# sun-huangqingbo/multiplexed-image-annotator

Measured on AMD Instinct MI355X. Metric: cells/sec annotated (whole node), higher is better.
Workload: dtype f16

## Files before the change

multiplexed-image-annotator_amd/csrc/cell_attention.hip:

```cpp

#include "gemm_epi.h"
#include "ribca_common.h"
#include "ribca_kernels.h"

namespace ribca {

namespace {

typedef __attribute__((__vector_size__(4 * sizeof(_Float16)))) _Float16 f16x4c;
typedef __attribute__((__vector_size__(4 * sizeof(short)))) short s16x4c;
__device__ __forceinline__ f16x4c lds_read_tr16c(const char* p) {
  return __builtin_bit_cast(f16x4c, __builtin_amdgcn_ds_read_tr16_b64_v4i16((s16x4c __attribute__((address_space(3)))*)(p)));
}

constexpr int kTP = 112, kVRows = 128;

template <int D, int HD> struct CellGeom {
  static constexpr int Dp = (D + 31) / 32 * 32;
  static constexpr int NK = Dp / 32;
  static constexpr int GD = HD == 32 ? 64 : 48;
  static constexpr int NTP = GD / 16;
  static constexpr int WROWS = 3 * GD;
  static constexpr int WSTAGE = WROWS * ROWB;
  static constexpr int GROUPS = D / GD;
  static constexpr int HPG = GD / HD;
  static constexpr int KIMG = kTP * ROWB;
  static constexpr int VROWB = 4 * GD;
  static constexpr int VIMG = kVRows * VROWB + 64;
  static constexpr int CB = 2 * 3 * D * 4;
  static constexpr int RING = 3;
  static constexpr int OFF_K = RING * WSTAGE;
  static constexpr int OFF_V = OFF_K + HPG * KIMG;
  static constexpr int OFF_CB = OFF_V + (VIMG + 15) / 16 * 16;
  static constexpr int LDS = OFF_CB + CB;
  static_assert(D % GD == 0 && GD % HD == 0 && HD % 4 == 0 && HD <= 32 && HPG % 2 == 0 && WROWS % 8 == 0, "head geometry");
};

}

template <int D, int HD>
__global__ __launch_bounds__(512) void cell_qkv_attention_kernel(const uint16_t* __restrict__ z, int ldz, const uint16_t* __restrict__ W, int ldw,
                                                                 const float* __restrict__ bias2, const float* __restrict__ csum,
                                                                 const float2* __restrict__ rowstat, uint16_t* __restrict__ out, int ldo, int T,
                                                                 float scale) {
  using G = CellGeom<D, HD>;
  constexpr int NK = G::NK, GROUPS = G::GROUPS, HPG = G::HPG, kRing = G::RING, kGroupDims = G::GD, NTP = G::NTP, kWStage = G::WSTAGE;
  constexpr int NTILES = 3 * NTP;
  constexpr int TOTAL = GROUPS * NK;
  constexpr int GPL = G::WROWS / 8;
  extern __shared__ __attribute__((aligned(16))) char smem[];
  const int tid = threadIdx.x, lane = tid & 63;
  const int wave = __builtin_amdgcn_readfirstlane(tid >> 6);
  const int cell = blockIdx.x;
  const int r16 = lane & 15, g = lane >> 4;

  for (int i = tid; i < 3 * D / 4; i += 512) {
    reinterpret_cast<float4*>(smem + G::OFF_CB)[i] = reinterpret_cast<const float4*>(csum)[i];
    reinterpret_cast<float4*>(smem + G::OFF_CB + 3 * D * 4)[i] = reinterpret_cast<const float4*>(bias2)[i];
  }
  for (int o = kTP * G::VROWB + tid * 16; o < G::VIMG; o += 512 * 16) *reinterpret_cast<uint4*>(smem + G::OFF_V + o) = uint4{0u, 0u, 0u, 0u};
  __syncthreads();

  if (wave == 7) {
    auto issue = [&](int step) {
      const int hg = step / NK, s = step - hg * NK;
      char* st = smem + (step % kRing) * kWStage;
#pragma unroll
      for (int i = 0; i < GPL; ++i) {
        const int row = i * 8 + (lane >> 3);
        const int which = row / kGroupDims, c = row - which * kGroupDims;
        const int n = which * D + hg * kGroupDims + c;
        const int ch = (lane & 7) ^ swz_f(row);
        const uint16_t* src = W + (size_t)n * ldw + s * (2 * BK) + ch * 8;
        __builtin_amdgcn_global_load_lds((const __attribute__((address_space(1))) void*)src, (__attribute__((address_space(3))) void*)(st + i * 1024), 16,
                                         0, 0);
      }
    };
    issue(0);
    issue(1);
    for (int step = 0; step < TOTAL; ++step) {
      if (step + 1 < TOTAL) wait_vmcnt<GPL>();
      else wait_vmcnt<0>();
      __builtin_amdgcn_s_barrier();
      asm volatile("" ::: "memory");
      if (step + 2 < TOTAL) issue(step + 2);
      if ((step + 1) % NK == 0) __builtin_amdgcn_s_barrier();
    }
    return;
  }

  const int tok = wave * 16 + r16;
  const int trow = tok < T ? tok : T - 1;
  const uint16_t* zr = z + ((size_t)cell * T + trow) * ldz;
  f16x8 ahi[NK], alo[NK];
#pragma unroll
  for (int s = 0; s < NK; ++s) {
    const uint4* p = reinterpret_cast<const uint4*>(zr + (4 * s + g) * 16);
    ahi[s] = __builtin_bit_cast(f16x8, p[0]);
    alo[s] = __builtin_bit_cast(f16x8, p[1]);
  }
  const float2 rs = rowstat[(size_t)cell * T + trow];
  const float rstd = rs.x, nm = -rs.y * rs.x;
  const char* cb = smem + G::OFF_CB;
  uint16_t* orow = out + ((size_t)cell * T + tok) * ldo;
  int w_rd[NTILES];
#pragma unroll
  for (int j = 0; j < NTILES; ++j) w_rd[j] = lds_off(16 * j + r16, 2 * g);
  const int k_wr = lds_off(tok, 2 * g);
  constexpr int KST = 4, NT = 7;

  int step = 0;
  for (int hg = 0; hg < GROUPS; ++hg) {
    f32x4 acc[NTILES];
#pragma unroll
    for (int j = 0; j < NTILES; ++j) acc[j] = f32x4{0.f, 0.f, 0.f, 0.f};
#pragma unroll
    for (int s = 0; s < NK; ++s, ++step) {
      asm volatile("s_waitcnt lgkmcnt(0)" ::: "memory");
      __builtin_amdgcn_s_barrier();
      asm volatile("" ::: "memory");
      const char* st = smem + (step % kRing) * kWStage;
#pragma unroll
      for (int jb = 0; jb < NTILES / 3; ++jb) {
        f16x8 whi[3], wlo[3];
#pragma unroll
        for (int j = 0; j < 3; ++j) {
          whi[j] = __builtin_bit_cast(f16x8, *reinterpret_cast<const uint4*>(st + w_rd[3 * jb + j]));
          wlo[j] = __builtin_bit_cast(f16x8, *reinterpret_cast<const uint4*>(st + (w_rd[3 * jb + j] ^ 16)));
        }
#pragma unroll
        for (int j = 0; j < 3; ++j) acc[3 * jb + j] = mfma_f16(wlo[j], ahi[s], acc[3 * jb + j]);
#pragma unroll
        for (int j = 0; j < 3; ++j) acc[3 * jb + j] = mfma_f16(whi[j], alo[s], acc[3 * jb + j]);
#pragma unroll
        for (int j = 0; j < 3; ++j) acc[3 * jb + j] = mfma_f16(whi[j], ahi[s], acc[3 * jb + j]);
      }
    }
#pragma unroll
    for (int j = 0; j < NTILES; ++j) {
      const int n = (j / NTP) * D + hg * kGroupDims + 16 * (j % NTP) + 4 * g;
      const float4 c4 = *reinterpret_cast<const float4*>(cb + n * 4), b4 = *reinterpret_cast<const float4*>(cb + 3 * D * 4 + n * 4);
      const f32x2v r2 = {rstd, rstd}, n2 = {nm, nm};
      const f32x2v lo2 = fma2(r2, f32x2v{acc[j][0], acc[j][1]}, fma2(n2, f32x2v{c4.x, c4.y}, f32x2v{b4.x, b4.y}));
      const f32x2v hi2 = fma2(r2, f32x2v{acc[j][2], acc[j][3]}, fma2(n2, f32x2v{c4.z, c4.w}, f32x2v{b4.z, b4.w}));
      acc[j] = f32x4{lo2.x, lo2.y, hi2.x, hi2.y};
    }
    f16x8 qhi[HPG], qlo[HPG];
#pragma unroll
    for (int h = 0; h < HPG; ++h) {
      constexpr int dummy = 0; (void)dummy;
      const int d_lo = h * HD, d_hi = d_lo + HD;
      const int tA = d_lo / 16, tB = (d_hi - 1) / 16;
      const bool inA = 16 * tA + 4 * g >= d_lo && 16 * tA + 4 * g < d_hi;
      const bool inB = tB != tA && 16 * tB + 4 * g >= d_lo && 16 * tB + 4 * g < d_hi;
      float qa[4], qb[4], ka[4], kb[4];
#pragma unroll
      for (int r = 0; r < 4; ++r) {
        qa[r] = inA ? acc[tA][r] * scale : 0.f;
        qb[r] = inB ? acc[tB][r] * scale : 0.f;
        ka[r] = inA ? acc[NTP + tA][r] : 0.f;
        kb[r] = inB ? acc[NTP + tB][r] : 0.f;
      }
      uint2 h0, l0, h1, l1;
      split4(qa, h0, l0);
      split4(qb, h1, l1);
      qhi[h] = __builtin_bit_cast(f16x8, uint4{h0.x, h0.y, h1.x, h1.y});
      qlo[h] = __builtin_bit_cast(f16x8, uint4{l0.x, l0.y, l1.x, l1.y});
      split4(ka, h0, l0);
      split4(kb, h1, l1);
      char* kimg = smem + G::OFF_K + h * G::KIMG;
      *reinterpret_cast<uint4*>(kimg + k_wr) = uint4{h0.x, h0.y, h1.x, h1.y};
      *reinterpret_cast<uint4*>(kimg + (k_wr ^ 16)) = uint4{l0.x, l0.y, l1.x, l1.y};
    }
    {
      uint16_t* vrow = reinterpret_cast<uint16_t*>(smem + G::OFF_V + tok * G::VROWB);
#pragma unroll
      for (int j = 0; j < NTP; ++j) {
        const float v4[4] = {acc[2 * NTP + j][0], acc[2 * NTP + j][1], acc[2 * NTP + j][2], acc[2 * NTP + j][3]};
        const int jj = kGroupDims == 64 ? (j ^ (tok & 3)) : j;
        ps_store4_pair<16>(vrow, 16 * jj + 4 * g, v4);
      }
    }
    asm volatile("s_waitcnt lgkmcnt(0)" ::: "memory");
    __builtin_amdgcn_s_barrier();
    asm volatile("" ::: "memory");

    constexpr int DT = (HD + 15) / 16;
    const char* vimg = smem + G::OFF_V;
#pragma unroll
    for (int hp = 0; hp < HPG; hp += 2) {
      f32x4 s[2][2 * KST];
#pragma unroll
      for (int kt = 0; kt < NT; ++kt) {
        const int ko = lds_off(16 * kt + r16, 2 * g);
#pragma unroll
        for (int e = 0; e < 2; ++e) {
          const char* kimg = smem + G::OFF_K + (hp + e) * G::KIMG;
          const f16x8 kh = __builtin_bit_cast(f16x8, *reinterpret_cast<const uint4*>(kimg + ko));
          const f16x8 kl = __builtin_bit_cast(f16x8, *reinterpret_cast<const uint4*>(kimg + (ko ^ 16)));
          s[e][kt] = f32x4{0.f, 0.f, 0.f, 0.f};
          s[e][kt] = mfma_f16(kl, qhi[hp + e], s[e][kt]);
          s[e][kt] = mfma_f16(kh, qlo[hp + e], s[e][kt]);
          s[e][kt] = mfma_f16(kh, qhi[hp + e], s[e][kt]);
        }
      }
      f16x8 phi[2][KST], plo[2][KST];
#pragma unroll
      for (int e = 0; e < 2; ++e) {
#pragma unroll
        for (int r = 0; r < 4; ++r)
          if (16 * (NT - 1) + 4 * g + r >= T) s[e][NT - 1][r] = -INFINITY;
        float mx = -INFINITY;
#pragma unroll
        for (int kt = 0; kt < NT; ++kt)
#pragma unroll
          for (int r = 0; r < 4; ++r) mx = fmaxf(mx, s[e][kt][r]);
        mx = fmaxf(mx, __shfl_xor(mx, 16, 64));
        mx = fmaxf(mx, __shfl_xor(mx, 32, 64));
        const f32x2v l2 = {1.44269504089f, 1.44269504089f}, moff = {-mx * 1.44269504089f, -mx * 1.44269504089f};
        f32x2v sum2 = {0.f, 0.f};
#pragma unroll
        for (int kt = 0; kt < NT; ++kt) {
          const f32x2v a0 = fma2(f32x2v{s[e][kt][0], s[e][kt][1]}, l2, moff);
          const f32x2v a1 = fma2(f32x2v{s[e][kt][2], s[e][kt][3]}, l2, moff);
          const f32x2v e0 = {__builtin_amdgcn_exp2f(a0.x), __builtin_amdgcn_exp2f(a0.y)}, e1 = {__builtin_amdgcn_exp2f(a1.x), __builtin_amdgcn_exp2f(a1.y)};
          s[e][kt] = f32x4{e0.x, e0.y, e1.x, e1.y};
          sum2 += e0;
          sum2 += e1;
        }
        float sum = sum2.x + sum2.y;
        sum += __shfl_xor(sum, 16, 64);
        sum += __shfl_xor(sum, 32, 64);
        const float inv = 1.0f / sum;
        const f32x2v inv2 = {inv, inv};
        s[e][NT] = f32x4{0.f, 0.f, 0.f, 0.f};
#pragma unroll
        for (int t = 0; t < KST; ++t) {
          const f32x2v pa0 = f32x2v{s[e][2 * t][0], s[e][2 * t][1]} * inv2, pa1 = f32x2v{s[e][2 * t][2], s[e][2 * t][3]} * inv2;
          const f32x2v pb0 = f32x2v{s[e][2 * t + 1][0], s[e][2 * t + 1][1]} * inv2, pb1 = f32x2v{s[e][2 * t + 1][2], s[e][2 * t + 1][3]} * inv2;
          const float pa[4] = {pa0.x, pa0.y, pa1.x, pa1.y}, pb[4] = {pb0.x, pb0.y, pb1.x, pb1.y};
          uint2 ha, la, hb, lb;
          split4_unit(pa, ha, la);
          split4_unit(pb, hb, lb);
          phi[e][t] = __builtin_bit_cast(f16x8, uint4{ha.x, ha.y, hb.x, hb.y});
          plo[e][t] = __builtin_bit_cast(f16x8, uint4{la.x, la.y, lb.x, lb.y});
        }
      }
#pragma unroll
      for (int dt = 0; dt < DT; ++dt) {
        f32x4 o[2] = {f32x4{0.f, 0.f, 0.f, 0.f}, f32x4{0.f, 0.f, 0.f, 0.f}};
#pragma unroll
        for (int t = 0; t < KST; ++t) {
#pragma unroll
          for (int e = 0; e < 2; ++e) {
            const int dcol0 = (hp + e) * HD + 16 * dt + 4 * (r16 & 3);
            const int dcol = kGroupDims == 64 ? ((((dcol0 >> 4) ^ (r16 >> 2)) << 4) | (dcol0 & 15)) : dcol0;
            const int voff = (dcol >> 3) * 32 + (dcol & 7) * 2;
            const char* va = vimg + (32 * t + 4 * g + (r16 >> 2)) * G::VROWB + voff;
            const f16x4c h0 = lds_read_tr16c(va), l0 = lds_read_tr16c(va + 16);
            const f16x4c h1 = lds_read_tr16c(va + 16 * G::VROWB), l1 = lds_read_tr16c(va + 16 * G::VROWB + 16);
            const f16x8 vhi = __builtin_shufflevector(h0, h1, 0, 1, 2, 3, 4, 5, 6, 7);
            const f16x8 vlo = __builtin_shufflevector(l0, l1, 0, 1, 2, 3, 4, 5, 6, 7);
            o[e] = mfma_f16(vlo, phi[e][t], o[e]);
            o[e] = mfma_f16(vhi, plo[e][t], o[e]);
            o[e] = mfma_f16(vhi, phi[e][t], o[e]);
          }
        }
        const int d = 16 * dt + 4 * g;
        if (tok < T && d < HD) {
#pragma unroll
          for (int e = 0; e < 2; ++e) {
            const float v4[4] = {o[e][0], o[e][1], o[e][2], o[e][3]};
            ps_store4(orow, (hg * HPG + hp + e) * HD + d, v4);
          }
        }
      }
    }
  }
}

bool cell_attention_supported(int D, int H, int T) { return H == kHeads && T == kTokens && (D == 144 || D == 288 || D == 384); }

void launch_cell_qkv_attention(const uint16_t* z, int ldz, const uint16_t* W, int ldw, const float* bias2, const float* csum, const float2* rowstat,
                               uint16_t* out, int ldo, int cells, int D, float scale, hipStream_t s) {
  if (cells <= 0) return;
  auto go = [&](auto kern, int lds) {
    static unsigned long long attr_done[3] = {0ull, 0ull, 0ull};
    const int slot = D == 288 ? 1 : D == 384 ? 2 : 0;
    if (!ensure_dynamic_lds(reinterpret_cast<const void*>(kern), lds, attr_done[slot])) return;
    hipLaunchKernelGGL(kern, dim3(cells), dim3(512), lds, s, z, ldz, W, ldw, bias2, csum, rowstat, out, ldo, (int)kTokens, scale);
  };
  if (D == 288) go(cell_qkv_attention_kernel<288, 24>, CellGeom<288, 24>::LDS);
  else if (D == 384) go(cell_qkv_attention_kernel<384, 32>, CellGeom<384, 32>::LDS);
  else go(cell_qkv_attention_kernel<144, 12>, CellGeom<144, 12>::LDS);
}

}
```

Baseline: 16910.

## Software-pipeline cell attention: interleave head softmax with other head's MFMA tiles

Restructures the per-head-pair attention loop so that the softmax of one head (max, exp, normalize, hi/lo split) is sliced into seven units and interleaved with the QK^T tiles of the second head and the PV tiles of the first. Explicit sched_group_barrier hints tell the compiler to alternate LDS reads, VALU, transcendental and MFMA instructions. This aims to hide the softmax VALU/exp latency behind matrix-core work. Cross-lane reductions also switch from shfl_xor to permlane16/32 swaps. The cost is higher register pressure from keeping two heads' scores and outputs live, plus hand-tuned schedule constants that may not fit every head geometry.

Result: no change. 16870 (-0.3%).

```diff
diff --git a/multiplexed-image-annotator_amd/csrc/cell_attention.hip b/multiplexed-image-annotator_amd/csrc/cell_attention.hip
--- a/multiplexed-image-annotator_amd/csrc/cell_attention.hip
+++ b/multiplexed-image-annotator_amd/csrc/cell_attention.hip
@@ -1,3 +1,6 @@
+
+#include <type_traits>
+#include <utility>
 
 #include "gemm_epi.h"
 #include "ribca_common.h"
@@ -36,6 +39,53 @@
   static_assert(D % GD == 0 && GD % HD == 0 && HD % 4 == 0 && HD <= 32 && HPG % 2 == 0 && WROWS % 8 == 0, "head geometry");
 };
 
+constexpr int kUnits = 7;
+constexpr int kSliceValu[kUnits] = {30, 26, 26, 50, 30, 30, 30};
+constexpr int kSliceTrans[kUnits] = {0, 12, 12, 5, 0, 0, 0};
+constexpr int pv_first(int u, int npv) { return (u * npv + kUnits / 2) / kUnits; }
+
+template <int... I, class F> __device__ __forceinline__ void static_for_impl(std::integer_sequence<int, I...>, F&& f) {
+  (f(std::integral_constant<int, I>{}), ...);
+}
+template <int N, class F> __device__ __forceinline__ void static_for(F&& f) { static_for_impl(std::make_integer_sequence<int, N>{}, f); }
+
+template <int NM, int NDS, int NV, int NTR> __device__ __forceinline__ void sched_unit() {
+  if constexpr (NM > 0) {
+    constexpr int lead = NV / 2, v = (NV - lead) / NM, tr = (NTR + NM - 1) / NM;
+    __builtin_amdgcn_sched_group_barrier(0x100, NDS, 0);
+    __builtin_amdgcn_sched_group_barrier(0x002, lead, 0);
+    static_for<NM>([](auto) __attribute__((always_inline)) {
+      __builtin_amdgcn_sched_group_barrier(0x008, 1, 0);
+      __builtin_amdgcn_sched_group_barrier(0x002, v, 0);
+      if constexpr (tr > 0) __builtin_amdgcn_sched_group_barrier(0x400, tr, 0);
+    });
+  }
+}
+template <int NT, int NDS, int NM> __device__ __forceinline__ void sched_tiles() {
+  __builtin_amdgcn_sched_group_barrier(0x100, NDS, 0);
+  static_for<NT>([](auto ic) __attribute__((always_inline)) {
+    if constexpr (decltype(ic)::value + 1 < NT) __builtin_amdgcn_sched_group_barrier(0x100, NDS, 0);
+    __builtin_amdgcn_sched_group_barrier(0x008, NM, 0);
+  });
+}
+
+__device__ __forceinline__ float xor16_max(float v) {
+  const auto r = __builtin_amdgcn_permlane16_swap(__float_as_uint(v), __float_as_uint(v), false, false);
+  return fmaxf(__uint_as_float(r[0]), __uint_as_float(r[1]));
+}
+__device__ __forceinline__ float xor16_sum(float v) {
+  const auto r = __builtin_amdgcn_permlane16_swap(__float_as_uint(v), __float_as_uint(v), false, false);
+  return __uint_as_float(r[0]) + __uint_as_float(r[1]);
+}
+__device__ __forceinline__ float xor32_max(float v) {
+  const auto r = __builtin_amdgcn_permlane32_swap(__float_as_uint(v), __float_as_uint(v), false, false);
+  return fmaxf(__uint_as_float(r[0]), __uint_as_float(r[1]));
+}
+__device__ __forceinline__ float xor32_sum(float v) {
+  const auto r = __builtin_amdgcn_permlane32_swap(__float_as_uint(v), __float_as_uint(v), false, false);
+  return __uint_as_float(r[0]) + __uint_as_float(r[1]);
+}
+
 }
 
 template <int D, int HD>
@@ -185,96 +235,122 @@
     __builtin_amdgcn_s_barrier();
     asm volatile("" ::: "memory");
 
-    constexpr int DT = (HD + 15) / 16;
+    constexpr int DT = (HD + 15) / 16, NPV = DT * KST;
     const char* vimg = smem + G::OFF_V;
 #pragma unroll
     for (int hp = 0; hp < HPG; hp += 2) {
-      f32x4 s[2][2 * KST];
-#pragma unroll
-      for (int kt = 0; kt < NT; ++kt) {
+      f32x4 s[2][2 * KST], o[2][DT];
+      f16x8 phi[2][KST], plo[2][KST];
+      float moff1[2], inv[2];
+      f32x2v sum2[2];
+      auto st_tile = [&](int e, int kt) __attribute__((always_inline)) {
         const int ko = lds_off(16 * kt + r16, 2 * g);
-#pragma unroll
-        for (int e = 0; e < 2; ++e) {
-          const char* kimg = smem + G::OFF_K + (hp + e) * G::KIMG;
-          const f16x8 kh = __builtin_bit_cast(f16x8, *reinterpret_cast<const uint4*>(kimg + ko));
-          const f16x8 kl = __builtin_bit_cast(f16x8, *reinterpret_cast<const uint4*>(kimg + (ko ^ 16)));
-          s[e][kt] = f32x4{0.f, 0.f, 0.f, 0.f};
-          s[e][kt] = mfma_f16(kl, qhi[hp + e], s[e][kt]);
-          s[e][kt] = mfma_f16(kh, qlo[hp + e], s[e][kt]);
-          s[e][kt] = mfma_f16(kh, qhi[hp + e], s[e][kt]);
+        const char* kimg = smem + G::OFF_K + (hp + e) * G::KIMG;
+        const f16x8 kh = __builtin_bit_cast(f16x8, *reinterpret_cast<const uint4*>(kimg + ko));
+        const f16x8 kl = __builtin_bit_cast(f16x8, *reinterpret_cast<const uint4*>(kimg + (ko ^ 16)));
+        s[e][kt] = f32x4{0.f, 0.f, 0.f, 0.f};
+        s[e][kt] = mfma_f16(kl, qhi[hp + e], s[e][kt]);
+        s[e][kt] = mfma_f16(kh, qlo[hp + e], s[e][kt]);
+        s[e][kt] = mfma_f16(kh, qhi[hp + e], s[e][kt]);
+      };
+      auto pv_tile = [&](int e, int i) __attribute__((always_inline)) {
+        const int dt = i / KST, t = i - dt * KST;
+        if (t == 0) o[e][dt] = f32x4{0.f, 0.f, 0.f, 0.f};
+        const int dcol0 = (hp + e) * HD + 16 * dt + 4 * (r16 & 3);
+        const int dcol = kGroupDims == 64 ? ((((dcol0 >> 4) ^ (r16 >> 2)) << 4) | (dcol0 & 15)) : dcol0;
+        const int voff = (dcol >> 3) * 32 + (dcol & 7) * 2;
+        const char* va = vimg + (32 * t + 4 * g + (r16 >> 2)) * G::VROWB + voff;
+        const f16x4c h0 = lds_read_tr16c(va), l0 = lds_read_tr16c(va + 16);
+        const f16x4c h1 = lds_read_tr16c(va + 16 * G::VROWB), l1 = lds_read_tr16c(va + 16 * G::VROWB + 16);
+        const f16x8 vhi = __builtin_shufflevector(h0, h1, 0, 1, 2, 3, 4, 5, 6, 7);
+        const f16x8 vlo = __builtin_shufflevector(l0, l1, 0, 1, 2, 3, 4, 5, 6, 7);
+        o[e][dt] = mfma_f16(vlo, phi[e][t], o[e][dt]);
+        o[e][dt] = mfma_f16(vhi, plo[e][t], o[e][dt]);
+        o[e][dt] = mfma_f16(vhi, phi[e][t], o[e][dt]);
+      };
+      auto exp_tile = [&](int e, int kt) __attribute__((always_inline)) {
+        const f32x2v l2 = {1.44269504089f, 1.44269504089f}, moff = {moff1[e], moff1[e]};
+        const f32x2v a0 = fma2(f32x2v{s[e][kt][0], s[e][kt][1]}, l2, moff);
+        const f32x2v a1 = fma2(f32x2v{s[e][kt][2], s[e][kt][3]}, l2, moff);
+        const f32x2v e0 = {__builtin_amdgcn_exp2f(a0.x), __builtin_amdgcn_exp2f(a0.y)}, e1 = {__builtin_amdgcn_exp2f(a1.x), __builtin_amdgcn_exp2f(a1.y)};
+        s[e][kt] = f32x4{e0.x, e0.y, e1.x, e1.y};
+        sum2[e] += e0;
+        sum2[e] += e1;
+      };
+      auto split_step = [&](int e, int t) __attribute__((always_inline)) {
+        const f32x2v inv2 = {inv[e], inv[e]};
+        const f32x2v pa0 = f32x2v{s[e][2 * t][0], s[e][2 * t][1]} * inv2, pa1 = f32x2v{s[e][2 * t][2], s[e][2 * t][3]} * inv2;
+        const f32x2v pb0 = f32x2v{s[e][2 * t + 1][0], s[e][2 * t + 1][1]} * inv2, pb1 = f32x2v{s[e][2 * t + 1][2], s[e][2 * t + 1][3]} * inv2;
+        const float pa[4] = {pa0.x, pa0.y, pa1.x, pa1.y}, pb[4] = {pb0.x, pb0.y, pb1.x, pb1.y};
+        uint2 ha, la, hb, lb;
+        split4_unit(pa, ha, la);
+        split4_unit(pb, hb, lb);
+        phi[e][t] = __builtin_bit_cast(f16x8, uint4{ha.x, ha.y, hb.x, hb.y});
+        plo[e][t] = __builtin_bit_cast(f16x8, uint4{la.x, la.y, lb.x, lb.y});
+      };
+      auto softmax_slice = [&](int e, int u) __attribute__((always_inline)) {
+        if (u == 0) {
+#pragma unroll
+          for (int r = 0; r < 4; ++r)
+            if (16 * (NT - 1) + 4 * g + r >= T) s[e][NT - 1][r] = -INFINITY;
+          float mx = -INFINITY;
+#pragma unroll
+          for (int kt = 0; kt < NT; ++kt)
+#pragma unroll
+            for (int r = 0; r < 4; ++r) mx = fmaxf(mx, s[e][kt][r]);
+          mx = xor32_max(xor16_max(mx));
+          moff1[e] = -mx * 1.44269504089f;
+          sum2[e] = f32x2v{0.f, 0.f};
+        } else if (u == 1 || u == 2) {
+#pragma unroll
+          for (int kt = 3 * (u - 1); kt < 3 * u; ++kt) exp_tile(e, kt);
+        } else if (u == 3) {
+          exp_tile(e, NT - 1);
+          float sum = sum2[e].x + sum2[e].y;
+          sum = xor32_sum(xor16_sum(sum));
+          inv[e] = 1.0f / sum;
+          s[e][NT] = f32x4{0.f, 0.f, 0.f, 0.f};
+          split_step(e, 0);
+        } else {
+          split_step(e, u - 3);
         }
-      }
-      f16x8 phi[2][KST], plo[2][KST];
-#pragma unroll
-      for (int e = 0; e < 2; ++e) {
-#pragma unroll
-        for (int r = 0; r < 4; ++r)
-          if (16 * (NT - 1) + 4 * g + r >= T) s[e][NT - 1][r] = -INFINITY;
-        float mx = -INFINITY;
-#pragma unroll
-        for (int kt = 0; kt < NT; ++kt)
-#pragma unroll
-          for (int r = 0; r < 4; ++r) mx = fmaxf(mx, s[e][kt][r]);
-        mx = fmaxf(mx, __shfl_xor(mx, 16, 64));
-        mx = fmaxf(mx, __shfl_xor(mx, 32, 64));
-        const f32x2v l2 = {1.44269504089f, 1.44269504089f}, moff = {-mx * 1.44269504089f, -mx * 1.44269504089f};
-        f32x2v sum2 = {0.f, 0.f};
-#pragma unroll
-        for (int kt = 0; kt < NT; ++kt) {
-          const f32x2v a0 = fma2(f32x2v{s[e][kt][0], s[e][kt][1]}, l2, moff);
-          const f32x2v a1 = fma2(f32x2v{s[e][kt][2], s[e][kt][3]}, l2, moff);
-          const f32x2v e0 = {__builtin_amdgcn_exp2f(a0.x), __builtin_amdgcn_exp2f(a0.y)}, e1 = {__builtin_amdgcn_exp2f(a1.x), __builtin_amdgcn_exp2f(a1.y)};
-          s[e][kt] = f32x4{e0.x, e0.y, e1.x, e1.y};
-          sum2 += e0;
-          sum2 += e1;
-        }
-        float sum = sum2.x + sum2.y;
-        sum += __shfl_xor(sum, 16, 64);
-        sum += __shfl_xor(sum, 32, 64);
-        const float inv = 1.0f / sum;
-        const f32x2v inv2 = {inv, inv};
-        s[e][NT] = f32x4{0.f, 0.f, 0.f, 0.f};
-#pragma unroll
-        for (int t = 0; t < KST; ++t) {
-          const f32x2v pa0 = f32x2v{s[e][2 * t][0], s[e][2 * t][1]} * inv2, pa1 = f32x2v{s[e][2 * t][2], s[e][2 * t][3]} * inv2;
-          const f32x2v pb0 = f32x2v{s[e][2 * t + 1][0], s[e][2 * t + 1][1]} * inv2, pb1 = f32x2v{s[e][2 * t + 1][2], s[e][2 * t + 1][3]} * inv2;
-          const float pa[4] = {pa0.x, pa0.y, pa1.x, pa1.y}, pb[4] = {pb0.x, pb0.y, pb1.x, pb1.y};
-          uint2 ha, la, hb, lb;
-          split4_unit(pa, ha, la);
-          split4_unit(pb, hb, lb);
-          phi[e][t] = __builtin_bit_cast(f16x8, uint4{ha.x, ha.y, hb.x, hb.y});
-          plo[e][t] = __builtin_bit_cast(f16x8, uint4{la.x, la.y, lb.x, lb.y});
-        }
-      }
+      };
+
+#pragma unroll
+      for (int kt = 0; kt < NT; ++kt) st_tile(0, kt);
+      sched_tiles<NT, 2, 3>();
+      __builtin_amdgcn_sched_barrier(0);
+      static_for<kUnits>([&](auto uc) __attribute__((always_inline)) {
+        constexpr int u = decltype(uc)::value;
+        st_tile(1, u);
+        softmax_slice(0, u);
+        sched_unit<3, 2, kSliceValu[u], kSliceTrans[u]>();
+        __builtin_amdgcn_sched_barrier(0);
+      });
+      static_for<kUnits>([&](auto uc) __attribute__((always_inline)) {
+        constexpr int u = decltype(uc)::value;
+        constexpr int i0 = pv_first(u, NPV), i1 = pv_first(u + 1, NPV);
+#pragma unroll
+        for (int i = i0; i < i1; ++i) pv_tile(0, i);
+        softmax_slice(1, u);
+        sched_unit<3 * (i1 - i0), 4 * (i1 - i0), kSliceValu[u], kSliceTrans[u]>();
+        __builtin_amdgcn_sched_barrier(0);
+      });
 #pragma unroll
       for (int dt = 0; dt < DT; ++dt) {
-        f32x4 o[2] = {f32x4{0.f, 0.f, 0.f, 0.f}, f32x4{0.f, 0.f, 0.f, 0.f}};
-#pragma unroll
-        for (int t = 0; t < KST; ++t) {
-#pragma unroll
-          for (int e = 0; e < 2; ++e) {
-            const int dcol0 = (hp + e) * HD + 16 * dt + 4 * (r16 & 3);
-            const int dcol = kGroupDims == 64 ? ((((dcol0 >> 4) ^ (r16 >> 2)) << 4) | (dcol0 & 15)) : dcol0;
-            const int voff = (dcol >> 3) * 32 + (dcol & 7) * 2;
-            const char* va = vimg + (32 * t + 4 * g + (r16 >> 2)) * G::VROWB + voff;
-            const f16x4c h0 = lds_read_tr16c(va), l0 = lds_read_tr16c(va + 16);
-            const f16x4c h1 = lds_read_tr16c(va + 16 * G::VROWB), l1 = lds_read_tr16c(va + 16 * G::VROWB + 16);
-            const f16x8 vhi = __builtin_shufflevector(h0, h1, 0, 1, 2, 3, 4, 5, 6, 7);
-            const f16x8 vlo = __builtin_shufflevector(l0, l1, 0, 1, 2, 3, 4, 5, 6, 7);
-            o[e] = mfma_f16(vlo, phi[e][t], o[e]);
-            o[e] = mfma_f16(vhi, plo[e][t], o[e]);
-            o[e] = mfma_f16(vhi, phi[e][t], o[e]);
-          }
-        }
+#pragma unroll
+        for (int t = 0; t < KST; ++t) pv_tile(1, dt * KST + t);
         const int d = 16 * dt + 4 * g;
         if (tok < T && d < HD) {
 #pragma unroll
           for (int e = 0; e < 2; ++e) {
-            const float v4[4] = {o[e][0], o[e][1], o[e][2], o[e][3]};
+            const float v4[4] = {o[e][dt][0], o[e][dt][1], o[e][dt][2], o[e][dt][3]};
             ps_store4(orow, (hg * HPG + hp + e) * HD + d, v4);
           }
         }
       }
+      sched_tiles<NPV, 4, 3>();
+      __builtin_amdgcn_sched_barrier(0);
     }
   }
 }
```
